# markweberdev/maskbit

Hardware: AMD Instinct MI355X
Metric: images/sec (256x256, 64-step MaskBit-12bit, CFG) (higher is better)
Workload: dtype f16

## Files before the change

### maskbit_amd/csrc/gemm_ht.hip

```cpp
#include <algorithm>

#include "mb_kernels.h"

namespace mb {

#define MB_SWZ(r) (((r) >> 1) & 7)

typedef int i32x4 __attribute__((ext_vector_type(4)));
typedef int i32x8 __attribute__((ext_vector_type(8)));
typedef h16 h16x16 __attribute__((ext_vector_type(16)));


template <int MT, int EPI, int XP = 0, bool SEQ = false, bool PAIR = false, int NS = 1>
__global__ __launch_bounds__(512, 2) void gemm_ht_kernel(GemmArgs a, int tiles_m, int tiles_n) {
  constexpr bool HN = NS > 1, QN = NS == 4;
  constexpr int NTW = 4 / NS;
  static_assert(NS == 1 || NS == 2 || NS == 4, "column split");
  static_assert(!HN || (SEQ && !PAIR && XP == 6 && EPI == EPI_RES_F32), "half-column tiles: plain sequence tiles with mini-tiles, residual epilogue");
  static_assert(!SEQ || MT == 8, "sequence-aligned tiles use the 256-row machinery");
  static_assert(XP == 0 || XP == 6, "fp16 K-tiles, optionally with mini-tiles");
  static_assert(!PAIR || SEQ, "pair tiles are sequence-aligned");
  constexpr bool MINI = XP == 6;
  static_assert(!MINI || SEQ, "mini-tile passes are written for sequence-aligned tiles");
  constexpr int MINI_A = 128 * 64, MINI_B = 256 * 64;
  constexpr bool PERSIST = true;
  constexpr int BM = 32 * MT, MH = MT / 2;
  constexpr int AH_ROWS = BM / 2;
  constexpr int AH_BYTES = AH_ROWS * 128, BH_BYTES = 128 * 128;
  constexpr int X_BYTES = SEQ ? 1024 : 0;
  constexpr int PAR_BYTES = 2 * AH_BYTES + 2 * BH_BYTES + X_BYTES;
  constexpr int MINI_OFF = 2 * PAR_BYTES;
  constexpr int A_INSTR = AH_ROWS / 8;
  extern __shared__ __attribute__((aligned(16))) char smem[];

  const int tid = threadIdx.x, lane = tid & 63;
  const int wave = __builtin_amdgcn_readfirstlane(tid >> 6);
  const int grp = wave >> 2;
  const int wm = wave >> 2, wn = wave & 3;
  const int l15 = lane & 15, g = lane >> 4;
  const int K = a.K, nk = K / 64;
  constexpr bool SPLIT = !PAIR;
  const int KA = SPLIT && a.kw ? a.kw : K, nka = KA / 64;
  const int KW = SPLIT && a.kw ? a.kw : K, nkw = KW / 64;
  const h16* const Alo = SPLIT && a.A2 ? a.A2 : a.A;
  const h16* const Wlo = a.W;
  const int SQ = a.seq_rows ? a.seq_rows : 257;
  const int tps_sh = 31 - __builtin_clz((unsigned)((SQ - 1) >> (PAIR ? 7 : 8)));
  const int TPS = 1 << tps_sh;
  const int ntiles = tiles_m * tiles_n;

  struct Plan {
    uint32_t offA[2][2], offB[2][2], offX;
    int m0, n0;
    int cls;
    int q;
    int seq;
    int hb;
  };
  int dstA[2], dstB[2];
#pragma unroll
  for (int j = 0; j < 2; ++j) { dstA[j] = min(wave + 8 * j, A_INSTR - 1) * 1024; dstB[j] = (QN ? (wave >> 1) * 4 + (wave & 1) : wave + 8 * j) * 1024; }
  auto make_plan = [&](int vb, Plan& p) {
    int lane_o = lane;
    asm volatile("" : "+v"(lane_o));
    const int L = xcd_remap(vb, ntiles);
    const int sr = L / (8 * tiles_n);
    const int rows_sr = min(8, tiles_m - sr * 8);
    const int rem = L - sr * 8 * tiles_n;
    const int tn = rem / rows_sr, tm = sr * 8 + (rem - tn * rows_sr);
    p.m0 = SEQ ? (tm >> tps_sh) * SQ + (tm & (TPS - 1)) * (PAIR ? 128 : 256) : tm * BM; p.n0 = (tn / NS) * 256;
    p.hb = tn % NS;
    p.cls = SEQ ? (tm >> tps_sh) * SQ + SQ - 1 : 0; p.q = SEQ ? tm & (TPS - 1) : 0;
    p.seq = SEQ ? tm >> tps_sh : tm;
#pragma unroll
    for (int j = 0; j < 2; ++j) {
      const int ja = min(wave + 8 * j, A_INSTR - 1);
      const int hra = ja * 8 + (lane_o >> 3);
      const int wms = hra / (8 * MT), r = hra - wms * (8 * MT);
      const int slot_a = (lane_o & 7) ^ MB_SWZ(hra);
      const int hrb = (QN ? (wave >> 1) * 4 + (wave & 1) : wave + 8 * j) * 8 + (lane_o >> 3);
      const int wns = hrb >> 5, c = hrb & 31;
      const int slot_b = (lane_o & 7) ^ MB_SWZ(hrb);
#pragma unroll
      for (int h = 0; h < 2; ++h) {
        const int gm = PAIR ? p.m0 + h * a.pair_rows + hra : min(p.m0 + wms * (16 * MT) + h * (8 * MT) + r, a.M - 1);
        p.offA[h][j] = (uint32_t)gm * (uint32_t)(2 * KA) + slot_a * 16;
        const int gn = min(p.n0 + wns * 64 + (HN ? p.hb * (64 / NS) : h * 32) + c, a.N - 1);
        p.offB[h][j] = (uint32_t)gn * (uint32_t)(2 * KW) + slot_b * 16;
      }
    }
    p.offX = (uint32_t)(PAIR ? p.cls + ((lane_o >> 3) == 1 ? a.pair_rows : 0) : min(p.cls, a.M - 1)) * (uint32_t)(2 * KA) + ((lane_o & 7) ^ MB_SWZ(lane_o >> 3)) * 16;
  };
  auto ktile_a = [&](int u) -> const char* { if constexpr (!SPLIT) return (const char*)a.A + u * 128; return (const char*)(u < nka ? a.A : Alo) + (u < nka ? u : u - nka) * 128; };
  auto ktile_w = [&](int u) -> const char* { if constexpr (!SPLIT) return (const char*)a.W + u * 128; return (const char*)(u < nkw ? a.W : Wlo) + (u < nkw ? u : u - nkw) * 128; };
  auto dma_x = [&](const Plan& p, const char* kp, int parb) {
    if (SEQ && wave == 7) MB_GLDS16_SB(kp, p.offX, smem + parb + 2 * AH_BYTES + 2 * BH_BYTES);
  };
  auto dma_a = [&](const Plan& p, const char* kp, int parb, int h) {
    char* buf = smem + parb + h * AH_BYTES;
#pragma unroll
    for (int j = 0; j < 2; ++j) {
      MB_GLDS16_SB2(kp, p.offA[h][j], buf, dstA[j]);
    }
  };
  auto dma_b = [&](const Plan& p, const char* kp, int parb, int h) {
    if (HN && h == 1) return;
    char* buf = smem + parb + 2 * AH_BYTES + h * BH_BYTES;
#pragma unroll
    for (int j = 0; j < (QN ? 1 : 2); ++j) {
      MB_GLDS16_SB2(kp, p.offB[h][j], buf, dstB[j]);
    }
  };
  const int KM = SPLIT && a.kw ? a.kw : K;
  const int nmk = KM / 128;
  const int nseq = PAIR ? a.pair_rows / SQ : a.M / SQ;
  const int grp_bytes = PAIR ? TPS * 128 : TPS * 256;
  const bool mini_every = MINI && (PAIR ? a.nlo == 2 : !a.kw);
  struct MiniPos { const uint8_t *a4, *w4, *xs, *ws; };
  const uint32_t ml_a = (uint32_t)((lane >> 2) * 2 * KM + (((lane & 3) ^ ((lane >> 3) & 3)) * 16));
  auto ml_w = [&]() -> uint32_t { int lo_ = lane; asm volatile("" : "+v"(lo_)); return (uint32_t)lo_ * 16; };
  const uint32_t ml_xs = (uint32_t)(lane >> 5) * (uint32_t)nseq * (uint32_t)grp_bytes + (lane & 15) * 4;
  auto ml_ws = [&]() -> uint32_t { int lo_ = lane; asm volatile("" : "+v"(lo_)); return (uint32_t)(lo_ & 15) * 4; };
  auto mini_pos = [&](const Plan& p) -> MiniPos {
    constexpr int si = 0, ps = 0;
    const int m0 = p.m0, n0 = p.n0, hb = p.hb, tq = p.q, sq = p.seq;
    const uint32_t row0 = PAIR ? m0 + wave * 16 : m0 + (wave >> 2) * 128 + ps * 64 + (wave & 3) * 16;
    const uint32_t wrow = QN ? wave * 4 + hb : HN ? (wave >> 1) * 4 + hb * 2 + (wave & 1) : wave;
    const uint32_t gq = PAIR ? tq * 2 + wm : tq * 4 + wm * 2 + ps;
    MiniPos m;
    m.a4 = a.lo[si].A4 + (size_t)row0 * 2 * KM;
    m.w4 = a.lo[si].W4 + (size_t)((n0 >> 4) + wrow) * nmk * 1024;
    m.xs = a.lo[si].a_scale + ((uint32_t)sq * (uint32_t)grp_bytes + gq * 64);
    m.ws = a.lo[si].w_scale + (uint32_t)(((n0 >> 6) + wn) * nmk) * 64;
    auto uni = [](const uint8_t* q) -> const uint8_t* {
      const uint64_t v = (uint64_t)q;
      return (const uint8_t*)(((uint64_t)(uint32_t)__builtin_amdgcn_readfirstlane((int)(v >> 32)) << 32) | (uint32_t)__builtin_amdgcn_readfirstlane((int)v));
    };
    m.a4 = uni(m.a4); m.w4 = uni(m.w4); m.xs = uni(m.xs); m.ws = uni(m.ws);
    return m;
  };
  const uint32_t xs_step = 2u * (uint32_t)nseq * (uint32_t)grp_bytes;
  auto mini_step = [&](MiniPos& m) { m.a4 += 64; m.w4 += 1024; m.xs += xs_step; m.ws += 64; };
  auto mini_switch = [&](MiniPos& m) {
    const size_t back = (size_t)nmk;
    if constexpr (PAIR) {
      auto ka = (const char __attribute__((address_space(4)))*)__builtin_amdgcn_kernarg_segment_ptr();
      asm volatile("" : "+s"(ka));
      auto l = (const GemmArgs::LoSet __attribute__((address_space(4)))*)(ka + offsetof(GemmArgs, lo));
      m.a4 += ((uintptr_t)l[1].A4 - (uintptr_t)l[0].A4) - back * 64;
      m.w4 += ((uintptr_t)l[1].W4 - (uintptr_t)l[0].W4) - back * 1024;
      m.xs += ((uintptr_t)l[1].a_scale - (uintptr_t)l[0].a_scale) - back * xs_step;
      m.ws += ((uintptr_t)l[1].w_scale - (uintptr_t)l[0].w_scale) - back * 64;
    } else {
      m.a4 += (size_t)64 * 2 * KM - back * 64;
      m.w4 -= back * 1024;
      m.xs += 64 - back * xs_step;
      m.ws -= back * 64;
    }
  };
  auto mini_dma_a = [&](const MiniPos& m) {
    MB_GLDS16_SB(m.a4, ml_a, smem + MINI_OFF + wave * 1024);
  };
  auto mini_dma_b = [&](const MiniPos& m) {
    if constexpr (QN) {
      if (wave < 4) MB_GLDS16_SB(m.w4, ml_w(), smem + MINI_OFF + MINI_A + wave * 1024);
      return;
    }
    if constexpr (HN) {
      MB_GLDS16_SB(m.w4, ml_w(), smem + MINI_OFF + MINI_A + wave * 1024);
      return;
    }
    const uint32_t mlw = ml_w();
#pragma unroll
    for (int jx = 0; jx < 2; ++jx)
      MB_GLDS16_SB(m.w4 + (size_t)(8 * jx) * nmk * 1024, mlw, smem + MINI_OFF + MINI_A + (wave + 8 * jx) * 1024);
  };
  int mws = 0, mxs = 0;
  auto mini_scale_issue = [&](const MiniPos& m) {
    asm volatile("global_load_dword %0, %1, %2" : "=v"(mxs) : "v"(ml_xs), "s"(m.xs) : "memory");
    asm volatile("global_load_dword %0, %1, %2" : "=v"(mws) : "v"(ml_ws()), "s"(m.ws) : "memory");
  };
  auto prologue_rest = [&](const Plan& p) {
    const char *a0 = ktile_a(0), *a1 = ktile_a(1), *w0 = ktile_w(0), *w1 = ktile_w(1);
    dma_a(p, a0, 0, 0); dma_b(p, w0, 0, 0); dma_b(p, w0, 0, 1); dma_a(p, a0, 0, 1);
    dma_a(p, a1, PAR_BYTES, 0); dma_b(p, w1, PAR_BYTES, 1); dma_a(p, a1, PAR_BYTES, 1); dma_b(p, w1, PAR_BYTES, 0);
  };
  auto prologue_x = [&](const Plan& p) { dma_x(p, ktile_a(0), 0); dma_x(p, ktile_a(1), PAR_BYTES); };
  auto prologue = [&](const Plan& p) { prologue_x(p); prologue_rest(p); if constexpr (MINI) { const MiniPos m0 = mini_pos(p); mini_dma_a(m0); mini_dma_b(m0); } };

  int foff[2], xoffe[2];
#pragma unroll
  for (int ks = 0; ks < 2; ++ks) {
    foff[ks] = l15 * 128 + (((ks * 4 + g) ^ MB_SWZ(l15)) * 16);
    xoffe[ks] = (l15 == 0 || (PAIR && l15 == 1)) ? 2 * AH_BYTES + 2 * BH_BYTES + foff[ks] : foff[ks];
  }
  const int mfo = (lane & 15) * 64 + (((lane >> 4) ^ ((lane >> 1) & 3)) * 16);
  const int xbase = wm * (8 * MT) * 128;
  const int wbase = 2 * AH_BYTES + wn * 32 * 128;

#define MB_LOAD_A(H)                                                                            \
  _Pragma("unroll") for (int i = 0; i < MH; ++i) _Pragma("unroll") for (int ks = 0; ks < 2; ++ks) \
      xa[i] = frag_set(xa[i], *(const h16x8*)(par + (H) * AH_BYTES + xbase + i * 16 * 128 + fo[ks]), ks);
#define MB_LOAD_B(H)                                                                            \
  _Pragma("unroll") for (int i = 0; i < (QN ? 1 : 2); ++i) _Pragma("unroll") for (int ks = 0; ks < 2; ++ks) \
      wb[H][i] = frag_set(wb[H][i], *(const h16x8*)(par + wbase + (H) * BH_BYTES + i * 16 * 128 + fo[ks]), ks);
#define MB_SYNC_L()                                     \
  __builtin_amdgcn_s_barrier();                         \
  __builtin_amdgcn_sched_barrier(0);                    \
  __builtin_amdgcn_s_setprio(1);
  auto frag_set = [](h16x16 f, h16x8 v, int ks) -> h16x16 {
    return ks == 0 ? __builtin_shufflevector(__builtin_shufflevector(v, v, 0, 1, 2, 3, 4, 5, 6, 7, 0, 1, 2, 3, 4, 5, 6, 7), f, 0, 1, 2, 3, 4, 5, 6, 7, 24, 25, 26, 27, 28, 29, 30, 31)
                   : __builtin_shufflevector(f, __builtin_shufflevector(v, v, 0, 1, 2, 3, 4, 5, 6, 7, 0, 1, 2, 3, 4, 5, 6, 7), 0, 1, 2, 3, 4, 5, 6, 7, 16, 17, 18, 19, 20, 21, 22, 23);
  };
  auto mma_tile = [&](f32x4 c, const h16x16& w, const h16x16& x) -> f32x4 {
    c = MB_MFMA_16x16x32(__builtin_shufflevector(w, w, 0, 1, 2, 3, 4, 5, 6, 7), __builtin_shufflevector(x, x, 0, 1, 2, 3, 4, 5, 6, 7), c);
    return MB_MFMA_16x16x32(__builtin_shufflevector(w, w, 8, 9, 10, 11, 12, 13, 14, 15), __builtin_shufflevector(x, x, 8, 9, 10, 11, 12, 13, 14, 15), c);
  };
#define MB_MMA_END                                                                                  \
  __builtin_amdgcn_s_setprio(0);                                                                    \
  __builtin_amdgcn_sched_barrier(0);                                                                \
  __builtin_amdgcn_s_barrier();
#define MB_MMA(AH, BH) MB_MMA_DO(AH, BH) MB_MMA_END
#define MB_MINI_ONE(AH, N, I)                                                                       \
  acc[N][(AH) * MH + (I)] = __builtin_amdgcn_mfma_scale_f32_16x16x128_f8f6f4(                        \
      __builtin_shufflevector(mwb[N], mwb[N], 0, 1, 2, 3, -1, -1, -1, -1), __builtin_shufflevector(mxa[I], mxa[I], 0, 1, 2, 3, -1, -1, -1, -1), \
      acc[N][(AH) * MH + (I)], 4, 4, N, mwsel, I, mxs);
#define MB_MINI_MMA_QN(AH)                                                                          \
  MB_MINI_ONE(AH, 0, 0) MB_MINI_ONE(AH, 0, 1) MB_MINI_ONE(AH, 0, 2) MB_MINI_ONE(AH, 0, 3)           \
  _Pragma("unroll") for (int i = 0; i < MH; ++i) asm volatile("" : "+v"(acc[0][(AH) * MH + i]));
#define MB_MINI_MMA_HN(AH)                                                                          \
  MB_MINI_ONE(AH, 0, 0) MB_MINI_ONE(AH, 1, 0) MB_MINI_ONE(AH, 0, 1) MB_MINI_ONE(AH, 1, 1)           \
  MB_MINI_ONE(AH, 0, 2) MB_MINI_ONE(AH, 1, 2) MB_MINI_ONE(AH, 0, 3) MB_MINI_ONE(AH, 1, 3)           \
  _Pragma("unroll") for (int i = 0; i < MH; ++i) _Pragma("unroll") for (int n = 0; n < 2; ++n)      \
    asm volatile("" : "+v"(acc[n][(AH) * MH + i]));
#define MB_MINI_MMA(AH)                                                                             \
  MB_MINI_ONE(AH, 0, 0) MB_MINI_ONE(AH, 1, 0) MB_MINI_ONE(AH, 2, 0) MB_MINI_ONE(AH, 3, 0)           \
  MB_MINI_ONE(AH, 0, 1) MB_MINI_ONE(AH, 1, 1) MB_MINI_ONE(AH, 2, 1) MB_MINI_ONE(AH, 3, 1)           \
  MB_MINI_ONE(AH, 0, 2) MB_MINI_ONE(AH, 1, 2) MB_MINI_ONE(AH, 2, 2) MB_MINI_ONE(AH, 3, 2)           \
  MB_MINI_ONE(AH, 0, 3) MB_MINI_ONE(AH, 1, 3) MB_MINI_ONE(AH, 2, 3) MB_MINI_ONE(AH, 3, 3)           \
  _Pragma("unroll") for (int i = 0; i < MH; ++i) _Pragma("unroll") for (int n = 0; n < 4; ++n)      \
    asm volatile("" : "+v"(acc[n][(AH) * MH + i]));
#define MB_MMA_DO(AH, BH)                                                                           \
  {                                                                                                 \
    _Pragma("unroll") for (int i = 0; i < MH; ++i) _Pragma("unroll") for (int n = 0; n < (QN ? 1 : 2); ++n)  \
      acc[(BH) * 2 + n][(AH) * MH + i] = mma_tile(acc[(BH) * 2 + n][(AH) * MH + i], wb[BH][n], xa[i]); \
  }

  Plan cur;
  int vb = blockIdx.x;
  make_plan(vb, cur);
  auto scales_load = [&](const Plan& p) {
    const MiniPos m0 = mini_pos(p);
    mws = *(const int*)(m0.ws + ml_ws());
    mxs = *(const int*)(m0.xs + ml_xs);
  };
  auto scales_pack = [&]() {
    if constexpr (MINI) { asm volatile("s_waitcnt vmcnt(0)" : "+v"(mws), "+v"(mxs) :: "memory"); return; }
  };
  if constexpr (MINI) scales_load(cur);
  prologue(cur);
  if constexpr (MINI) scales_pack();
  else asm volatile("s_waitcnt vmcnt(0)" ::: "memory");
  __builtin_amdgcn_s_barrier();

  while (true) {
    f32x4 acc[4][MT];
#pragma unroll
    for (int i = 0; i < 4; ++i)
#pragma unroll
      for (int j = 0; j < MT; ++j) acc[i][j] = f32x4{0.f, 0.f, 0.f, 0.f};
    f32x4 acce[2] = {f32x4{0.f, 0.f, 0.f, 0.f}, f32x4{0.f, 0.f, 0.f, 0.f}};
    const bool cls_on = __builtin_amdgcn_readfirstlane(cur.q) == TPS - 1;
    h16x16 xa[MH], wb[2][2];

    MiniPos mp = {};
    if constexpr (MINI) { mp = mini_pos(cur); mini_step(mp); }
    if (grp == 1) __builtin_amdgcn_s_barrier();
#define MB_KTILE MB_KTILE_(0)
#define MB_KTILE_(MAH)               \
    {                                                                                                    \
      const char* par = smem + parb; \
      int fo[2], xo[2]; \
      _Pragma("unroll") for (int ks = 0; ks < 2; ++ks) { fo[ks] = foff[ks]; xo[ks] = xoffe[ks]; } \
       \
       \
       \
      const bool n1 = t >= 1 && t + 1 < nk, n2 = t + 2 < nk; \
       \
      MB_LOAD_B(0) MB_LOAD_A(0)                           \
      h16x16 xe; \
      if (SEQ && wm == 0 && cls_on) { xe = frag_set(xe, *(const h16x8*)(par + xo[0]), 0); xe = frag_set(xe, *(const h16x8*)(par + xo[1]), 1); } \
      MB_SYNC_L() \
      if (SEQ && wm == 0 && cls_on) { _Pragma("unroll") for (int n = 0; n < (QN ? 1 : 2); ++n) acce[n] = mma_tile(acce[n], wb[0][n], xe); } \
      MB_MMA_DO(0, 0) MB_MMA_END \
       \
      if constexpr (!HN) { MB_LOAD_B(1) } \
      if (!HN && SEQ && wm == 1 && cls_on) { xe = frag_set(xe, *(const h16x8*)(par + xo[0]), 0); xe = frag_set(xe, *(const h16x8*)(par + xo[1]), 1); } \
       \
      const bool mini_issue = MINI && t >= 1 && mdue != 0; \
      if (MINI && mini_issue) { if (mj == nmk) mini_switch(mp); mini_scale_issue(mp); mini_dma_a(mp); } \
      if (n1) dma_a(cur, pa1, PAR_BYTES - parb, 1); \
      MB_SYNC_L() \
      if (!HN && SEQ && wm == 1 && cls_on) { _Pragma("unroll") for (int n = 0; n < 2; ++n) acce[n] = mma_tile(acce[n], wb[1][n], xe); } \
      if constexpr (!HN) { MB_MMA_DO(0, 1) } MB_MMA_END \
       \
      MB_LOAD_A(1) \
      if (MINI && mini_issue) { mini_dma_b(mp); mini_step(mp); ++mj; } \
      if (n2) dma_a(cur, pa2, parb, 0); \
      MB_SYNC_L() if (!HN) { MB_MMA_DO(1, 1) } MB_MMA_END \
       \
       \
       \
      if (n2) { dma_b(cur, pw2, parb, 1); dma_x(cur, pa2, parb); dma_b(cur, pw2, parb, 0); } \
      if (t >= 1) { \
        if (MINI) {                                \
           \
           \
          const int wsel = __builtin_amdgcn_readfirstlane(n2 ? (wave == 7 ? 2 : 1) : 0); \
          if constexpr (QN)                               \
            asm volatile("s_cmp_eq_u32 %[w], 0\n\ts_cbranch_scc1 1f\n\ts_cmp_eq_u32 %[w], 1\n\ts_cbranch_scc1 2f\n\ts_waitcnt vmcnt(4)\n\ts_branch 3f\n" \
                         "1:\n\ts_waitcnt vmcnt(0)\n\ts_branch 3f\n2:\n\ts_waitcnt vmcnt(3)\n3:" \
                         : "+v"(mxs), "+v"(mws) : [w] "s"(wsel) : "memory", "scc"); \
          else if constexpr (HN)                          \
            asm volatile("s_cmp_eq_u32 %[w], 0\n\ts_cbranch_scc1 1f\n\ts_cmp_eq_u32 %[w], 1\n\ts_cbranch_scc1 2f\n\ts_waitcnt vmcnt(5)\n\ts_branch 3f\n" \
                         "1:\n\ts_waitcnt vmcnt(0)\n\ts_branch 3f\n2:\n\ts_waitcnt vmcnt(4)\n3:" \
                         : "+v"(mxs), "+v"(mws) : [w] "s"(wsel) : "memory", "scc"); \
          else \
          asm volatile("s_cmp_eq_u32 %[w], 0\n\ts_cbranch_scc1 1f\n\ts_cmp_eq_u32 %[w], 1\n\ts_cbranch_scc1 2f\n\ts_waitcnt vmcnt(7)\n\ts_branch 3f\n" \
                       "1:\n\ts_waitcnt vmcnt(0)\n\ts_branch 3f\n2:\n\ts_waitcnt vmcnt(6)\n3:" \
                       : "+v"(mxs), "+v"(mws) : [w] "s"(wsel) : "memory", "scc"); \
        } else if (n2) {                                  \
          if (SEQ && wave == 7) asm volatile("s_waitcnt vmcnt(7)" ::: "memory"); \
          else asm volatile("s_waitcnt vmcnt(6)" ::: "memory"); \
        } else asm volatile("s_waitcnt vmcnt(0)" ::: "memory"); \
      } \
      MB_SYNC_L() MB_MMA_DO(1, 0) MB_MMA_END \
       \
      if constexpr (MINI) { \
        if (mrun != 0) { \
          int mfo_ = mfo; \
          asm volatile("" : "+v"(mfo_)); \
          const char* mbuf = smem + MINI_OFF + mfo_; \
          i32x4 mxa[4], mwb[4]; \
          _Pragma("unroll") for (int n = 0; n < NTW; ++n) mwb[n] = *(const i32x4*)(mbuf + MINI_A + (wn * (64 / NS) + n * 16) * 64); \
          _Pragma("unroll") for (int i = 0; i < 4; ++i) mxa[i] = *(const i32x4*)(mbuf + (wm * 64 + i * 16) * 64); \
          const int mwsel = HN ? (int)((uint32_t)mws >> ((32 / NS) * cur.hb)) : mws;    \
          MB_SYNC_L() \
          if constexpr (QN) { MB_MINI_MMA_QN(MAH) } else if constexpr (HN) { MB_MINI_MMA_HN(MAH) } else { MB_MINI_MMA(MAH) } \
           \
          asm volatile("s_nop 15\n\ts_nop 15" ::: "memory"); \
          MB_MMA_END \
        } \
      } \
       \
      pa1 = pa2; \
      pa2 = SPLIT && t + 3 == nka ? (const char*)Alo : pa2 + 128; \
      pw2 = SPLIT && t + 3 == nkw ? (const char*)Wlo : pw2 + 128; \
      parb = PAR_BYTES - parb; \
      mdue ^= mflip; mrun ^= mflip; \
    }
    {
      int t = 0;
      int parb = 0;
      const char *pa1 = ktile_a(1), *pa2 = ktile_a(2), *pw2 = ktile_w(2);
      const int mflip = mini_every ? 0 : 1;
      int mdue = 1, mrun = mini_every ? 1 : 0, mj = 1;
      (void)mj;
      if constexpr (MINI && !PAIR) {
        for (; t < nk / 2; ++t) MB_KTILE_(0)
        for (; t < nk; ++t) MB_KTILE_(1)
      } else {
        for (; t < nk; ++t) MB_KTILE
      }
    }
#undef MB_KTILE
#undef MB_KTILE_
    if (grp == 0) __builtin_amdgcn_s_barrier();

    const float* __restrict__ resp = a.residual;
    float* __restrict__ out32 = a.out_f32;
    h16* __restrict__ out16 = a.out_h16;
    const int m0 = cur.m0, n0 = cur.n0, clsrow = cur.cls, tq = cur.q;
    constexpr int NROWS = SEQ ? MT + 1 : MT;
    int l15e = l15, ge = g;
    asm volatile("" : "+v"(l15e), "+v"(ge));
    auto row_of = [&](int r) {
      if (PAIR) return r < MT ? m0 + (r / MH) * a.pair_rows + wm * 64 + (r % MH) * 16 + l15e : clsrow + (l15e == 1 ? a.pair_rows : 0);
      return r < MT ? m0 + wm * (16 * MT) + (r / MH) * (8 * MT) + (r % MH) * 16 + l15e : clsrow;
    };
    auto col_of = [&](int r, int nt) {
      if (HN) return n0 + wn * 64 + cur.hb * (64 / NS) + (nt & (NTW - 1)) * 16 + ge * 4;
      return r < MT ? n0 + wn * 64 + (nt >> 1) * 32 + (nt & 1) * 16 + ge * 4 : n0 + wn * 64 + wm * 32 + nt * 16 + ge * 4;
    };
    auto row_ok = [&](int r) {
      if (PAIR) return r < MT ? true : (l15e < 2 && tq == TPS - 1);
      return r < MT ? row_of(r) < (SEQ ? m0 + 256 : a.M) : (l15e == 0 && (!HN || wm == 0) && tq == TPS - 1);
    };
    const int nvb = vb + gridDim.x;
    const bool has_next = PERSIST && nvb < ntiles;
    Plan nxt;
    if (has_next) { make_plan(nvb, nxt); prologue_x(nxt); }
    f32x4 bias4[4], bcls[2];
    if constexpr (MINI) {
#pragma unroll
      for (int nt = 0; nt < 4; ++nt) bias4[nt] = *(const f32x4*)(a.bias + col_of(0, nt));
      if (SEQ) { bcls[0] = *(const f32x4*)(a.bias + col_of(MT, 0)); bcls[1] = *(const f32x4*)(a.bias + col_of(MT, 1)); }
      else { bcls[0] = bias4[0]; bcls[1] = bias4[1]; }
      if (has_next) scales_load(nxt);
      asm volatile("s_waitcnt vmcnt(0)" : "+v"(bias4[0]), "+v"(bias4[1]), "+v"(bias4[2]), "+v"(bias4[3]), "+v"(bcls[0]), "+v"(bcls[1]) :: "memory");
      if (has_next) scales_pack();
      if (has_next) { prologue_rest(nxt); const MiniPos m0 = mini_pos(nxt); mini_dma_a(m0); mini_dma_b(m0); }
    } else {
#define MB_LDG16(dst, ptr) asm volatile("global_load_dwordx4 %0, %1, off" : "=v"(dst) : "v"(ptr) : "memory")
#pragma unroll
    for (int nt = 0; nt < 4; ++nt) MB_LDG16(bias4[nt], a.bias + col_of(0, nt));
    if (SEQ) { MB_LDG16(bcls[0], a.bias + col_of(MT, 0)); MB_LDG16(bcls[1], a.bias + col_of(MT, 1)); }
    else { bcls[0] = bias4[0]; bcls[1] = bias4[1]; }
#undef MB_LDG16
    if (has_next) prologue_rest(nxt);
    {
      const int hn = __builtin_amdgcn_readfirstlane(has_next ? 1 : 0);
      asm volatile("s_cmp_lg_u32 %[hn], 0\n\ts_cbranch_scc1 1f\n\ts_waitcnt vmcnt(0)\n1:\n\ts_waitcnt vmcnt(16)"
                   : "+v"(bias4[0]), "+v"(bias4[1]), "+v"(bias4[2]), "+v"(bias4[3]), "+v"(bcls[0]), "+v"(bcls[1])
                   : [hn] "s"(hn) : "memory", "scc");
    }
    }

    if constexpr (PAIR) {
      const float osc = a.scale ? *a.scale : 1.0f;
      auto pair2 = [&](f32x4& c, f32x4& dl, const f32x4& b) {
        f32x4 vc = __builtin_elementwise_fma(c, (f32x4)(osc), b);
        f32x4 vu = __builtin_elementwise_fma(dl, (f32x4)(osc), vc);
        if (EPI == EPI_GELU_H16 || EPI == EPI_GELU_F32) {
          const f32x2 c0 = gelu_erf2((f32x2){vc[0], vc[1]}), c1 = gelu_erf2((f32x2){vc[2], vc[3]});
          const f32x2 u0 = gelu_erf2((f32x2){vu[0], vu[1]}), u1 = gelu_erf2((f32x2){vu[2], vu[3]});
          vc = f32x4{c0.x, c0.y, c1.x, c1.y};
          vu = f32x4{u0.x - c0.x, u0.y - c0.y, u1.x - c1.x, u1.y - c1.y};
        }
        c = vc; dl = vu;
        asm volatile("" : "+v"(c), "+v"(dl));
      };
#pragma unroll
      for (int i = 0; i < MH; ++i)
#pragma unroll
        for (int nt = 0; nt < 4; ++nt) pair2(acc[nt][i], acc[nt][i + MH], bias4[nt]);
#pragma unroll
      for (int n = 0; n < 2; ++n) {
        f32x4 cup;
#pragma unroll
        for (int e = 0; e < 4; ++e) cup[e] = __shfl_up(acce[n][e], 1);
        f32x4 c = l15e == 1 ? cup : acce[n], dl = l15e == 1 ? acce[n] : f32x4{0.f, 0.f, 0.f, 0.f};
        pair2(c, dl, bcls[n]);
        acce[n] = l15e == 1 ? dl : c;
      }
    } else {
      const float osc = a.scale ? *a.scale : 1.0f;
#pragma unroll
      for (int r = 0; r < NROWS; ++r) {
        const int nn = r < MT ? NTW : (QN ? 1 : 2);
#pragma unroll
        for (int nt = 0; nt < nn; ++nt) {
          f32x4& c = r < MT ? acc[nt][r < MT ? r : 0] : acce[nt & 1];
          c = __builtin_elementwise_fma(c, (f32x4)(osc), r < MT ? bias4[nt] : bcls[nt & 1]);
          if (EPI == EPI_GELU_H16 || EPI == EPI_GELU_F32) {
            const f32x2 lo = gelu_erf2((f32x2){c[0], c[1]}), hi = gelu_erf2((f32x2){c[2], c[3]});
            c[0] = lo.x; c[1] = lo.y; c[2] = hi.x; c[3] = hi.y;
          }
          asm volatile("" : "+v"(c));
        }
      }
    }
    if (has_next) asm volatile("s_waitcnt vmcnt(0)" ::: "memory");
    if constexpr (SEQ && EPI == EPI_GELU_H16) {
      if (a.out4) {
        const uint32_t blk = (uint32_t)(n0 >> 6) + wn;
        const uint32_t nsq = (uint32_t)(PAIR ? a.pair_rows : a.M) / (uint32_t)SQ;
        const uint32_t ngrp = (uint32_t)TPS * (PAIR ? 2 : 4);
        auto emit4 = [&](uint32_t p0, uint32_t p1, uint32_t p2, uint32_t p3, uint8_t* dst, uint32_t row) {
          const auto sw = __builtin_amdgcn_permlane16_swap((p0 & 0xffffu) | (p2 << 16), (p1 & 0xffffu) | (p3 << 16), false, false);
          const uint32_t q0 = __builtin_amdgcn_perm(sw[1], sw[0], 0x05040100u);
          const uint32_t q1 = __builtin_amdgcn_perm(sw[1], sw[0], 0x07060302u);
          const auto sx = __builtin_amdgcn_permlane32_swap(q0, q1, false, false);
          *(uint2*)(dst + (size_t)row * 2 * a.N + ((n0 + wn * 64) >> 1) + (ge >> 1) * 16 + (ge & 1) * 8) = make_uint2(sx[0], sx[1]);
        };
#pragma unroll
        for (int hh = 0; hh < (PAIR ? 1 : 2); ++hh) {
          uint32_t sc4 = 0, sl4 = 0;
#pragma unroll
          for (int ii = 0; ii < MH; ++ii) {
            const int i = hh * MH + ii;
            float am = 0.f;
#pragma unroll
            for (int nt = 0; nt < 4; ++nt)
#pragma unroll
              for (int e = 0; e < 4; ++e) am = fmaxf(am, fabsf(acc[nt][i][e]));
            am = rows_max(am);
            const float mul = fp4_scale_mul_nosat(am);
            const uint32_t row = (uint32_t)row_of(i);
            sc4 |= fp4_scale_byte_nosat(am) << (8 * ii);
            emit4(fp4_pack4(acc[0][i][0], acc[0][i][1], acc[0][i][2], acc[0][i][3], mul), fp4_pack4(acc[1][i][0], acc[1][i][1], acc[1][i][2], acc[1][i][3], mul),
                  fp4_pack4(acc[2][i][0], acc[2][i][1], acc[2][i][2], acc[2][i][3], mul), fp4_pack4(acc[3][i][0], acc[3][i][1], acc[3][i][2], acc[3][i][3], mul),
                  a.out4, row);
            if (a.out4l) {
              f32x4 l[4];
              float aml = 0.f;
#pragma unroll
              for (int nt = 0; nt < 4; ++nt)
#pragma unroll
                for (int e = 0; e < 4; ++e) { l[nt][e] = acc[nt][i][e] - (float)to_h(acc[nt][i][e]); aml = fmaxf(aml, fabsf(l[nt][e])); }
              aml = rows_max(aml);
              const float mull = fp4_scale_mul_nosat(aml);
              sl4 |= fp4_scale_byte_nosat(aml) << (8 * ii);
              emit4(fp4_pack4(l[0][0], l[0][1], l[0][2], l[0][3], mull), fp4_pack4(l[1][0], l[1][1], l[1][2], l[1][3], mull),
                    fp4_pack4(l[2][0], l[2][1], l[2][2], l[2][3], mull), fp4_pack4(l[3][0], l[3][1], l[3][2], l[3][3], mull), a.out4l, row);
            }
          }
          const uint32_t gq = PAIR ? (uint32_t)tq * 2 + wm : (uint32_t)tq * 4 + wm * 2 + hh;
          if (ge == 0) ((uint32_t*)a.out4_scale)[((blk * nsq + (uint32_t)cur.seq) * ngrp + gq) * 16 + l15e] = sc4;
          if (ge == 0 && a.out4l) ((uint32_t*)a.out4l_scale)[((blk * nsq + (uint32_t)cur.seq) * ngrp + gq) * 16 + l15e] = sl4;
        }
      }
    }
    if (EPI == EPI_RES_F32) {
      const bool lnres = a.ln_stats != nullptr;
      constexpr int RB = (PAIR && MINI) ? 1 : 2;
      constexpr int NB = MT / RB;
      static_assert(MT % RB == 0, "whole batches");
      constexpr int NQ = QN ? 1 : 2;
      float4 rv[RB][2];
      float2 sv[RB] = {};
      auto fetch = [&](int k) {
        const int p = k / NB, r0 = (k % NB) * RB;
#pragma unroll
        for (int j = 0; j < RB; ++j) {
          const uint32_t rowc = (uint32_t)min(row_of(r0 + j), a.M - 1);
#pragma unroll
          for (int q = 0; q < NQ; ++q) rv[j][q] = *(const float4*)((const char*)resp + (size_t)((rowc * (uint32_t)a.N + (uint32_t)col_of(r0 + j, 2 * p + q)) * 4u));
          if (lnres) sv[j] = *(const float2*)(a.ln_stats + 2 * (size_t)rowc);
        }
      };
      auto add_one = [&](f32x4& c, const float4& rr, const float2& st, const f32x4& gm, const f32x4& bt) {
        if (lnres) {
          c[0] += ln_affine(rr.x, st.x, st.y, gm[0], bt[0]); c[1] += ln_affine(rr.y, st.x, st.y, gm[1], bt[1]);
          c[2] += ln_affine(rr.z, st.x, st.y, gm[2], bt[2]); c[3] += ln_affine(rr.w, st.x, st.y, gm[3], bt[3]);
        } else { c[0] += rr.x; c[1] += rr.y; c[2] += rr.z; c[3] += rr.w; }
      };
      f32x4 gm[2] = {}, bt[2] = {};
      auto affine = [&](int p) {
        if (lnres) {
#pragma unroll
          for (int q = 0; q < NQ; ++q) { gm[q] = *(const f32x4*)(a.ln_g + col_of(0, 2 * p + q)); bt[q] = *(const f32x4*)(a.ln_b + col_of(0, 2 * p + q)); }
        }
      };
      auto add = [&](int k) {
        const int p = k / NB, r0 = (k % NB) * RB;
#pragma unroll
        for (int j = 0; j < RB; ++j)
#pragma unroll
          for (int q = 0; q < NQ; ++q) add_one(acc[2 * p + q][r0 + j], rv[j][q], sv[j], gm[q], bt[q]);
      };
      auto store_one = [&](const f32x4& c, int r, int nt) {
        *(float4*)((char*)out32 + (size_t)(((uint32_t)row_of(r) * (uint32_t)a.N + (uint32_t)col_of(r, nt)) * 4u)) = make_float4(c[0], c[1], c[2], c[3]);
      };
      auto store = [&](int k) {
        const int p = k / NB, r0 = (k % NB) * RB;
#pragma unroll
        for (int j = 0; j < RB; ++j)
          if (row_ok(r0 + j)) {
#pragma unroll
            for (int q = 0; q < NQ; ++q) store_one(acc[2 * p + q][r0 + j], r0 + j, 2 * p + q);
          }
      };
      affine(0);
      fetch(0);
      constexpr int NSWEEP = HN ? 1 : 2;
#pragma unroll
      for (int k = 0; k < NSWEEP * NB; ++k) {
        asm volatile("" ::: "memory");
        add(k);
        if (k + 1 < NSWEEP * NB) { if ((k + 1) % NB == 0) affine((k + 1) / NB); fetch(k + 1); }
        asm volatile("" ::: "memory");
        store(k);
      }
      if (SEQ) {
        float4 rr[2]; float2 st = {};
        const uint32_t rowc = (uint32_t)min(row_of(MT), a.M - 1);
#pragma unroll
        for (int q = 0; q < NQ; ++q) {
          rr[q] = *(const float4*)((const char*)resp + (size_t)((rowc * (uint32_t)a.N + (uint32_t)col_of(MT, q)) * 4u));
          if (lnres) { gm[q] = *(const f32x4*)(a.ln_g + col_of(MT, q)); bt[q] = *(const f32x4*)(a.ln_b + col_of(MT, q)); }
        }
        if (lnres) st = *(const float2*)(a.ln_stats + 2 * (size_t)rowc);
#pragma unroll
        for (int q = 0; q < NQ; ++q) add_one(acce[q], rr[q], st, gm[q], bt[q]);
        if (row_ok(MT)) {
#pragma unroll
          for (int q = 0; q < NQ; ++q) store_one(acce[q], MT, q);
        }
      }
    } else {
      float satm = 0.f;
      bool satnan = false;
#pragma unroll
      for (int r = 0; r < NROWS; ++r) {
        const bool ok = row_ok(r);
        const int nn = r < MT ? 4 : 2;
        if (EPI == EPI_H16 || EPI == EPI_GELU_H16) {
#pragma unroll
          for (int pr = 0; pr < nn / 2; ++pr) {
            const f32x4 ca = r < MT ? acc[2 * pr][r < MT ? r : 0] : acce[0];
            const f32x4 cb = r < MT ? acc[2 * pr + 1][r < MT ? r : 0] : acce[1];
            if (a.sat && ok) {
              satm = fmaxf(fmaxf(satm, fmaxf(fmaxf(fabsf(ca[0]), fabsf(ca[1])), fmaxf(fabsf(ca[2]), fabsf(ca[3])))),
                           fmaxf(fmaxf(fabsf(cb[0]), fabsf(cb[1])), fmaxf(fabsf(cb[2]), fabsf(cb[3]))));
              const float sm = (ca[0] + ca[1]) + (ca[2] + ca[3]) + (cb[0] + cb[1]) + (cb[2] + cb[3]);
              satnan |= sm != sm;
            }
            const h16x2 ta0 = {to_h(ca[0]), to_h(ca[1])}, ta1 = {to_h(ca[2]), to_h(ca[3])};
            const h16x2 tb0 = {to_h(cb[0]), to_h(cb[1])}, tb1 = {to_h(cb[2]), to_h(cb[3])};
            const auto s0 = __builtin_amdgcn_permlane16_swap(__builtin_bit_cast(uint32_t, ta0), __builtin_bit_cast(uint32_t, tb0), false, false);
            const auto s1 = __builtin_amdgcn_permlane16_swap(__builtin_bit_cast(uint32_t, ta1), __builtin_bit_cast(uint32_t, tb1), false, false);
            const int n = col_of(r, 2 * pr + (ge & 1)) - (ge & 1) * 4;
            const size_t ob = (size_t)(((uint32_t)row_of(r) * (uint32_t)a.N + (uint32_t)n) * 2u);
            if (ok) *(uint4*)((char*)out16 + ob) = make_uint4(s0[0], s1[0], s0[1], s1[1]);
          }
        } else if (ok) {
#pragma unroll
          for (int nt = 0; nt < 4; ++nt)
            if (nt < nn) {
              const f32x4 c = r < MT ? acc[nt][r < MT ? r : 0] : acce[nt & 1];
              *(float4*)((char*)out32 + (size_t)(((uint32_t)row_of(r) * (uint32_t)a.N + (uint32_t)col_of(r, nt)) * 4u)) = make_float4(c[0], c[1], c[2], c[3]);
            }
        }
      }
      if ((EPI == EPI_H16 || EPI == EPI_GELU_H16) && a.sat && (satnan || !(satm <= MB_H16_MAX))) atomicAdd(a.sat, 1u);
    }
    if (has_next) __builtin_amdgcn_s_barrier();
    if (!has_next) break;
    cur = nxt;
    vb = nvb;
  }
#undef MB_LOAD_A
#undef MB_LOAD_B
#undef MB_SYNC_L
#undef MB_MMA
#undef MB_MMA_DO
#undef MB_MMA_END
#undef MB_MINI_ONE
#undef MB_MINI_MMA
#undef MB_MINI_MMA_HN
#undef MB_MINI_MMA_QN
}

static int g_cu_override = 0;
void set_cu_count(int n) { g_cu_override = n > 0 ? n : 0; }
static int num_cu_cached() {
  static int num_cu = 0;
  if (g_cu_override) return g_cu_override;
  if (!num_cu) {
    int dev = 0;
    (void)hipGetDevice(&dev);
    (void)hipDeviceGetAttribute(&num_cu, hipDeviceAttributeMultiprocessorCount, dev);
    if (num_cu <= 0) num_cu = 256;
  }
  return num_cu;
}

template <int MT, int EPI, int XP = 0, bool SEQ = false, bool PAIR = false, int NS = 1>
static void launch_ht(hipStream_t s, const GemmArgs& a, bool persistent = true) {
  constexpr int BM = 32 * MT;
  constexpr int LDS = 2 * (BM * 128 + 2 * 128 * 128 + (SEQ ? 1024 : 0)) + (XP == 6 ? 128 * 64 + 256 * 64 : 0);
  static bool configured = false;
  if (!configured) {
    (void)hipFuncSetAttribute((const void*)gemm_ht_kernel<MT, EPI, XP, SEQ, PAIR, NS>, hipFuncAttributeMaxDynamicSharedMemorySize, LDS);
    configured = true;
  }
  const int sq_rows = a.seq_rows ? a.seq_rows : 257;
  const int tiles_m = PAIR ? (a.pair_rows / sq_rows) * ((sq_rows - 1) / 128) : (SEQ ? (a.M / sq_rows) * ((sq_rows - 1) / 256) : (a.M + BM - 1) / BM), tiles_n = (a.N / 256) * NS;
  const int grid = persistent ? std::min(tiles_m * tiles_n, num_cu_cached()) : tiles_m * tiles_n;
  hipLaunchKernelGGL((gemm_ht_kernel<MT, EPI, XP, SEQ, PAIR, NS>), dim3(grid), dim3(512), LDS, s, a, tiles_m, tiles_n);
}

bool gemm_ht_supported(GemmEpi epi, const GemmArgs& a) {
  const int sqr = a.seq_rows ? a.seq_rows : 257;
  const int tok = a.pair_rows ? 128 : 256;
  if (a.seq_rows && ((sqr - 1) % tok || ((sqr - 1) / tok & ((sqr - 1) / tok - 1)) || (!a.pair_rows && a.M % sqr))) return false;
  if (a.pair_rows && (a.pair_rows % sqr || a.M != 2 * a.pair_rows || a.A2 || a.kw || epi == EPI_GELU_F32)) return false;
  if (a.nlo && (a.nlo > 2 || (a.pair_rows ? a.pair_rows % sqr : a.M % sqr) || (a.kw ? a.kw : a.K) % 128 || (!a.pair_rows && a.nlo != 1) ||
                ((a.A2 || a.kw) && (a.pair_rows || !a.A2 || a.K != 2 * a.kw)) ||
                !a.lo[0].A4 || !a.lo[0].W4 || !a.lo[0].a_scale || !a.lo[0].w_scale ||
                (a.nlo == 2 && (!a.lo[1].A4 || !a.lo[1].W4 || !a.lo[1].a_scale || !a.lo[1].w_scale)) || (uint64_t)a.M * a.K * 2 >= (1ull << 32) ||
                epi == EPI_GELU_F32)) return false;
  return epi != EPI_LOGITS_F32 && a.N % 256 == 0 && a.K % 64 == 0 && a.K >= 128 && (a.M >= 512 || a.nlo) &&
         (uint64_t)a.M * a.K * 2 < (1ull << 32) && (uint64_t)a.N * a.K * 2 < (1ull << 32) &&
         (uint64_t)a.M * a.N * 4 < (1ull << 32);
}

void gemm_ht(hipStream_t s, GemmEpi epi, const GemmArgs& a, int mt) {
  bool persistent = true;
  const int sqr = a.seq_rows ? a.seq_rows : 257;
  const long seq_tiles = (long)(a.M / sqr) * ((sqr - 1) / 256);
  if (mt >= 1000) { persistent = false; mt -= 1000; }
  if (mt != 6 && mt != 8 && mt != 257) {
    const int num_cu = num_cu_cached();
    auto cost = [&](int m) {
      const long tiles = (long)((a.M + 32 * m - 1) / (32 * m)) * (a.N / 256);
      return (double)((tiles + num_cu - 1) / num_cu) * 32 * m * (m == 8 ? 1.0 : 1.04);
    };
    mt = cost(8) <= cost(6) ? 8 : 6;
    if (a.M % sqr == 0) {
      const long tiles = (long)(a.M / sqr) * ((sqr - 1) / 256) * (a.N / 256);
      if ((double)((tiles + num_cu - 1) / num_cu) * 272 < cost(mt)) mt = 257;
    }
  }
  if (a.nlo) {
    switch (epi) {
      case EPI_H16: if (a.pair_rows) launch_ht<8, EPI_H16, 6, true, true>(s, a, persistent); else launch_ht<8, EPI_H16, 6, true>(s, a, persistent); break;
      case EPI_GELU_H16: if (a.pair_rows) launch_ht<8, EPI_GELU_H16, 6, true, true>(s, a, persistent); else launch_ht<8, EPI_GELU_H16, 6, true>(s, a, persistent); break;
      case EPI_RES_F32:
        if (a.pair_rows) launch_ht<8, EPI_RES_F32, 6, true, true>(s, a, persistent);
        else if (seq_tiles * (a.N / 256) * 4 <= num_cu_cached()) launch_ht<8, EPI_RES_F32, 6, true, false, 4>(s, a, persistent);
        else if (seq_tiles * (a.N / 256) * 2 <= num_cu_cached()) launch_ht<8, EPI_RES_F32, 6, true, false, 2>(s, a, persistent);
        else launch_ht<8, EPI_RES_F32, 6, true>(s, a, persistent);
        break;
      default: break;
    }
    return;
  }
  if (a.pair_rows) {
    switch (epi) {
      case EPI_H16: launch_ht<8, EPI_H16, 0, true, true>(s, a, persistent); break;
      case EPI_GELU_H16: launch_ht<8, EPI_GELU_H16, 0, true, true>(s, a, persistent); break;
      case EPI_RES_F32: launch_ht<8, EPI_RES_F32, 0, true, true>(s, a, persistent); break;
      default: break;
    }
    return;
  }
#define MB_HT_CASE(E)                                                      \
  case E:                                                                  \
    if (mt == 257) launch_ht<8, E, 0, true>(s, a, persistent);             \
    else if (mt == 8) launch_ht<8, E>(s, a, persistent);                   \
    else launch_ht<6, E>(s, a, persistent);                                \
    break;
  switch (epi) {
    MB_HT_CASE(EPI_H16) MB_HT_CASE(EPI_GELU_H16) MB_HT_CASE(EPI_RES_F32) MB_HT_CASE(EPI_GELU_F32)
    default: break;
  }
#undef MB_HT_CASE
}

}
```

Before: 34.70.

## Pipeline fp16 epilogue row by row with direct stores and relaxed waits

For sequence-aligned fp16 and GELU-fp16 epilogues, bias, GELU, optional fp4 packing and the fp16 stores now run row by row. Stores go out through inline global_store with scalar base pointers and permlane16 swaps that build 16-byte writes. The full vmcnt(0) wait before the epilogue becomes a computed partial wait, so next-tile prefetch loads keep flowing while stores drain. This cuts epilogue latency and register pressure, but relies on exact hand-counted vmcnt values, and the CLS bias now comes from bias4 instead of separate loads.

```diff
diff --git a/maskbit_amd/csrc/gemm_ht.hip b/maskbit_amd/csrc/gemm_ht.hip
--- a/maskbit_amd/csrc/gemm_ht.hip
+++ b/maskbit_amd/csrc/gemm_ht.hip
@@ -6,6 +6,7 @@
 
 #define MB_SWZ(r) (((r) >> 1) & 7)
 
+typedef int i32x2 __attribute__((ext_vector_type(2)));
 typedef int i32x4 __attribute__((ext_vector_type(4)));
 typedef int i32x8 __attribute__((ext_vector_type(8)));
 typedef h16 h16x16 __attribute__((ext_vector_type(16)));
@@ -21,6 +22,7 @@
   static_assert(XP == 0 || XP == 6, "fp16 K-tiles, optionally with mini-tiles");
   static_assert(!PAIR || SEQ, "pair tiles are sequence-aligned");
   constexpr bool MINI = XP == 6;
+  constexpr bool ROWPIPE = SEQ && (EPI == EPI_H16 || EPI == EPI_GELU_H16);
   static_assert(!MINI || SEQ, "mini-tile passes are written for sequence-aligned tiles");
   constexpr int MINI_A = 128 * 64, MINI_B = 256 * 64;
   constexpr bool PERSIST = true;
@@ -72,6 +74,10 @@
     p.hb = tn % NS;
     p.cls = SEQ ? (tm >> tps_sh) * SQ + SQ - 1 : 0; p.q = SEQ ? tm & (TPS - 1) : 0;
     p.seq = SEQ ? tm >> tps_sh : tm;
+    if constexpr (ROWPIPE) {
+      p.m0 = __builtin_amdgcn_readfirstlane(p.m0); p.n0 = __builtin_amdgcn_readfirstlane(p.n0); p.cls = __builtin_amdgcn_readfirstlane(p.cls);
+      p.q = __builtin_amdgcn_readfirstlane(p.q); p.seq = __builtin_amdgcn_readfirstlane(p.seq);
+    }
 #pragma unroll
     for (int j = 0; j < 2; ++j) {
       const int ja = min(wave + 8 * j, A_INSTR - 1);
@@ -404,7 +410,7 @@
     if constexpr (MINI) {
 #pragma unroll
       for (int nt = 0; nt < 4; ++nt) bias4[nt] = *(const f32x4*)(a.bias + col_of(0, nt));
-      if (SEQ) { bcls[0] = *(const f32x4*)(a.bias + col_of(MT, 0)); bcls[1] = *(const f32x4*)(a.bias + col_of(MT, 1)); }
+      if (SEQ && !ROWPIPE) { bcls[0] = *(const f32x4*)(a.bias + col_of(MT, 0)); bcls[1] = *(const f32x4*)(a.bias + col_of(MT, 1)); }
       else { bcls[0] = bias4[0]; bcls[1] = bias4[1]; }
       if (has_next) scales_load(nxt);
       asm volatile("s_waitcnt vmcnt(0)" : "+v"(bias4[0]), "+v"(bias4[1]), "+v"(bias4[2]), "+v"(bias4[3]), "+v"(bcls[0]), "+v"(bcls[1]) :: "memory");
@@ -414,7 +420,7 @@
 #define MB_LDG16(dst, ptr) asm volatile("global_load_dwordx4 %0, %1, off" : "=v"(dst) : "v"(ptr) : "memory")
 #pragma unroll
     for (int nt = 0; nt < 4; ++nt) MB_LDG16(bias4[nt], a.bias + col_of(0, nt));
-    if (SEQ) { MB_LDG16(bcls[0], a.bias + col_of(MT, 0)); MB_LDG16(bcls[1], a.bias + col_of(MT, 1)); }
+    if (SEQ && !ROWPIPE) { MB_LDG16(bcls[0], a.bias + col_of(MT, 0)); MB_LDG16(bcls[1], a.bias + col_of(MT, 1)); }
     else { bcls[0] = bias4[0]; bcls[1] = bias4[1]; }
 #undef MB_LDG16
     if (has_next) prologue_rest(nxt);
@@ -426,24 +432,28 @@
     }
     }
 
-    if constexpr (PAIR) {
-      const float osc = a.scale ? *a.scale : 1.0f;
-      auto pair2 = [&](f32x4& c, f32x4& dl, const f32x4& b) {
-        f32x4 vc = __builtin_elementwise_fma(c, (f32x4)(osc), b);
-        f32x4 vu = __builtin_elementwise_fma(dl, (f32x4)(osc), vc);
-        if (EPI == EPI_GELU_H16 || EPI == EPI_GELU_F32) {
-          const f32x2 c0 = gelu_erf2((f32x2){vc[0], vc[1]}), c1 = gelu_erf2((f32x2){vc[2], vc[3]});
-          const f32x2 u0 = gelu_erf2((f32x2){vu[0], vu[1]}), u1 = gelu_erf2((f32x2){vu[2], vu[3]});
-          vc = f32x4{c0.x, c0.y, c1.x, c1.y};
-          vu = f32x4{u0.x - c0.x, u0.y - c0.y, u1.x - c1.x, u1.y - c1.y};
-        }
-        c = vc; dl = vu;
-        asm volatile("" : "+v"(c), "+v"(dl));
-      };
-#pragma unroll
-      for (int i = 0; i < MH; ++i)
-#pragma unroll
-        for (int nt = 0; nt < 4; ++nt) pair2(acc[nt][i], acc[nt][i + MH], bias4[nt]);
+    const float osc = a.scale ? *a.scale : 1.0f;
+    auto pair2 = [&](f32x4& c, f32x4& dl, const f32x4& b) {
+      f32x4 vc = __builtin_elementwise_fma(c, (f32x4)(osc), b);
+      f32x4 vu = __builtin_elementwise_fma(dl, (f32x4)(osc), vc);
+      if (EPI == EPI_GELU_H16 || EPI == EPI_GELU_F32) {
+        const f32x2 c0 = gelu_erf2((f32x2){vc[0], vc[1]}), c1 = gelu_erf2((f32x2){vc[2], vc[3]});
+        const f32x2 u0 = gelu_erf2((f32x2){vu[0], vu[1]}), u1 = gelu_erf2((f32x2){vu[2], vu[3]});
+        vc = f32x4{c0.x, c0.y, c1.x, c1.y};
+        vu = f32x4{u0.x - c0.x, u0.y - c0.y, u1.x - c1.x, u1.y - c1.y};
+      }
+      c = vc; dl = vu;
+      asm volatile("" : "+v"(c), "+v"(dl));
+    };
+    auto plain1 = [&](f32x4& c, const f32x4& b) {
+      c = __builtin_elementwise_fma(c, (f32x4)(osc), b);
+      if (EPI == EPI_GELU_H16 || EPI == EPI_GELU_F32) {
+        const f32x2 lo = gelu_erf2((f32x2){c[0], c[1]}), hi = gelu_erf2((f32x2){c[2], c[3]});
+        c[0] = lo.x; c[1] = lo.y; c[2] = hi.x; c[3] = hi.y;
+      }
+      asm volatile("" : "+v"(c));
+    };
+    auto pair_cls = [&]() {
 #pragma unroll
       for (int n = 0; n < 2; ++n) {
         f32x4 cup;
@@ -453,75 +463,131 @@
         pair2(c, dl, bcls[n]);
         acce[n] = l15e == 1 ? dl : c;
       }
+    };
+    (void)pair2; (void)plain1; (void)pair_cls;
+    if constexpr (ROWPIPE) {
+      constexpr int NE4 = PAIR ? MH + 1 : MT + 2;
+      const bool o4 = EPI == EPI_GELU_H16 && a.out4 != nullptr, o4l = o4 && a.out4l != nullptr;
+      float satm = 0.f;
+      bool satnan = false;
+      auto store16 = [&](int r, int pr, const f32x4& ca, const f32x4& cb, bool lane_ok) {
+        if (a.sat && lane_ok) {
+          satm = fmaxf(fmaxf(satm, fmaxf(fmaxf(fabsf(ca[0]), fabsf(ca[1])), fmaxf(fabsf(ca[2]), fabsf(ca[3])))),
+                       fmaxf(fmaxf(fabsf(cb[0]), fabsf(cb[1])), fmaxf(fabsf(cb[2]), fabsf(cb[3]))));
+          const float sm = (ca[0] + ca[1]) + (ca[2] + ca[3]) + (cb[0] + cb[1]) + (cb[2] + cb[3]);
+          satnan |= sm != sm;
+        }
+        const h16x2 ta0 = {to_h(ca[0]), to_h(ca[1])}, ta1 = {to_h(ca[2]), to_h(ca[3])};
+        const h16x2 tb0 = {to_h(cb[0]), to_h(cb[1])}, tb1 = {to_h(cb[2]), to_h(cb[3])};
+        const auto s0 = __builtin_amdgcn_permlane16_swap(__builtin_bit_cast(uint32_t, ta0), __builtin_bit_cast(uint32_t, tb0), false, false);
+        const auto s1 = __builtin_amdgcn_permlane16_swap(__builtin_bit_cast(uint32_t, ta1), __builtin_bit_cast(uint32_t, tb1), false, false);
+        const int n = col_of(r, 2 * pr + (ge & 1)) - (ge & 1) * 4;
+        const uint32_t ob = ((uint32_t)row_of(r) * (uint32_t)a.N + (uint32_t)n) * 2u;
+        const i32x4 v = {(int)s0[0], (int)s1[0], (int)s0[1], (int)s1[1]};
+        if (lane_ok) asm volatile("s_nop 4\n\tglobal_store_dwordx4 %0, %1, %2\n\ts_nop 1" :: "v"(ob), "v"(v), "s"(out16) : "memory");
+      };
+      const uint32_t blk = (uint32_t)(n0 >> 6) + wn;
+      const uint32_t nsq = (uint32_t)(PAIR ? a.pair_rows : a.M) / (uint32_t)SQ;
+      const uint32_t ngrp = (uint32_t)TPS * (PAIR ? 2 : 4);
+      auto emit4 = [&](uint32_t p0, uint32_t p1, uint32_t p2, uint32_t p3, uint8_t* dst, uint32_t row) {
+        const auto sw = __builtin_amdgcn_permlane16_swap((p0 & 0xffffu) | (p2 << 16), (p1 & 0xffffu) | (p3 << 16), false, false);
+        const uint32_t q0 = __builtin_amdgcn_perm(sw[1], sw[0], 0x05040100u);
+        const uint32_t q1 = __builtin_amdgcn_perm(sw[1], sw[0], 0x07060302u);
+        const auto sx = __builtin_amdgcn_permlane32_swap(q0, q1, false, false);
+        const uint32_t ob = row * 2u * (uint32_t)a.N + (uint32_t)(((n0 + wn * 64) >> 1) + (ge >> 1) * 16 + (ge & 1) * 8);
+        const i32x2 v = {(int)sx[0], (int)sx[1]};
+        asm volatile("s_nop 4\n\tglobal_store_dwordx2 %0, %1, %2" :: "v"(ob), "v"(v), "s"(dst) : "memory");
+      };
+      uint32_t sc4 = 0, sl4 = 0;
+      auto e2m1_row = [&](int i) {
+        const int ii = i % MH;
+        float am = 0.f;
+#pragma unroll
+        for (int nt = 0; nt < 4; ++nt)
+#pragma unroll
+          for (int e = 0; e < 4; ++e) am = fmaxf(am, fabsf(acc[nt][i][e]));
+        am = rows_max(am);
+        const float mul = fp4_scale_mul_nosat(am);
+        const uint32_t row = (uint32_t)row_of(i);
+        sc4 |= fp4_scale_byte_nosat(am) << (8 * ii);
+        emit4(fp4_pack4(acc[0][i][0], acc[0][i][1], acc[0][i][2], acc[0][i][3], mul), fp4_pack4(acc[1][i][0], acc[1][i][1], acc[1][i][2], acc[1][i][3], mul),
+              fp4_pack4(acc[2][i][0], acc[2][i][1], acc[2][i][2], acc[2][i][3], mul), fp4_pack4(acc[3][i][0], acc[3][i][1], acc[3][i][2], acc[3][i][3], mul),
+              a.out4, row);
+        if (o4l) {
+          f32x4 l[4];
+          float aml = 0.f;
+#pragma unroll
+          for (int nt = 0; nt < 4; ++nt)
+#pragma unroll
+            for (int e = 0; e < 4; ++e) { l[nt][e] = acc[nt][i][e] - (float)to_h(acc[nt][i][e]); aml = fmaxf(aml, fabsf(l[nt][e])); }
+          aml = rows_max(aml);
+          const float mull = fp4_scale_mul_nosat(aml);
+          sl4 |= fp4_scale_byte_nosat(aml) << (8 * ii);
+          emit4(fp4_pack4(l[0][0], l[0][1], l[0][2], l[0][3], mull), fp4_pack4(l[1][0], l[1][1], l[1][2], l[1][3], mull),
+                fp4_pack4(l[2][0], l[2][1], l[2][2], l[2][3], mull), fp4_pack4(l[3][0], l[3][1], l[3][2], l[3][3], mull), a.out4l, row);
+        }
+        if (ii == MH - 1) {
+          const int hh = i / MH;
+          const uint32_t gq = PAIR ? (uint32_t)tq * 2 + wm : (uint32_t)tq * 4 + wm * 2 + hh;
+          const uint32_t sb = (((blk * nsq + (uint32_t)cur.seq) * ngrp + gq) * 16 + l15e) * 4u;
+          if (ge == 0) asm volatile("s_nop 4\n\tglobal_store_dword %0, %1, %2" :: "v"(sb), "v"(sc4), "s"(a.out4_scale) : "memory");
+          if (o4l) { if (ge == 0) asm volatile("s_nop 4\n\tglobal_store_dword %0, %1, %2" :: "v"(sb), "v"(sl4), "s"(a.out4l_scale) : "memory"); }
+          sc4 = 0; sl4 = 0;
+        }
+      };
+#pragma unroll
+      for (int i = 0; i < (PAIR ? MH : MT); ++i) {
+#pragma unroll
+        for (int nt = 0; nt < 4; ++nt) {
+          if constexpr (PAIR) pair2(acc[nt][i], acc[nt][i + MH], bias4[nt]);
+          else plain1(acc[nt][i], bias4[nt]);
+        }
+        if (o4) e2m1_row(i);
+#pragma unroll
+        for (int pr = 0; pr < 2; ++pr) store16(i, pr, acc[2 * pr][i], acc[2 * pr + 1][i], true);
+        if constexpr (PAIR) {
+#pragma unroll
+          for (int pr = 0; pr < 2; ++pr) store16(i + MH, pr, acc[2 * pr][i + MH], acc[2 * pr + 1][i + MH], true);
+        }
+      }
+      if (cls_on) {
+        bcls[0] = wm ? bias4[2] : bias4[0]; bcls[1] = wm ? bias4[3] : bias4[1];
+        if constexpr (PAIR) pair_cls();
+        else { plain1(acce[0], bcls[0]); plain1(acce[1], bcls[1]); }
+        store16(MT, 0, acce[0], acce[1], PAIR ? l15e < 2 : l15e == 0);
+      }
+      if (has_next) {
+        const int wsel = __builtin_amdgcn_readfirstlane((cls_on ? 1 : 0) + (o4 ? (o4l ? 4 : 2) : 0));
+        asm volatile("s_cmp_eq_u32 %[w], 0\n\ts_cbranch_scc1 10f\n\ts_cmp_eq_u32 %[w], 1\n\ts_cbranch_scc1 11f\n\t"
+                     "s_cmp_eq_u32 %[w], 2\n\ts_cbranch_scc1 12f\n\ts_cmp_eq_u32 %[w], 3\n\ts_cbranch_scc1 13f\n\t"
+                     "s_cmp_eq_u32 %[w], 4\n\ts_cbranch_scc1 14f\n\t"
+                     "s_waitcnt vmcnt(%[c5])\n\ts_branch 19f\n"
+                     "10:\n\ts_waitcnt vmcnt(%[c0])\n\ts_branch 19f\n11:\n\ts_waitcnt vmcnt(%[c1])\n\ts_branch 19f\n"
+                     "12:\n\ts_waitcnt vmcnt(%[c2])\n\ts_branch 19f\n13:\n\ts_waitcnt vmcnt(%[c3])\n\ts_branch 19f\n"
+                     "14:\n\ts_waitcnt vmcnt(%[c4])\n19:"
+                     :: [w] "s"(wsel), [c0] "n"(16), [c1] "n"(17), [c2] "n"(16 + NE4), [c3] "n"(17 + NE4), [c4] "n"(16 + 2 * NE4), [c5] "n"(17 + 2 * NE4)
+                     : "memory", "scc");
+      }
+      if (a.sat && (satnan || !(satm <= MB_H16_MAX))) atomicAdd(a.sat, 1u);
     } else {
-      const float osc = a.scale ? *a.scale : 1.0f;
-#pragma unroll
-      for (int r = 0; r < NROWS; ++r) {
-        const int nn = r < MT ? NTW : (QN ? 1 : 2);
-#pragma unroll
-        for (int nt = 0; nt < nn; ++nt) {
-          f32x4& c = r < MT ? acc[nt][r < MT ? r : 0] : acce[nt & 1];
-          c = __builtin_elementwise_fma(c, (f32x4)(osc), r < MT ? bias4[nt] : bcls[nt & 1]);
-          if (EPI == EPI_GELU_H16 || EPI == EPI_GELU_F32) {
-            const f32x2 lo = gelu_erf2((f32x2){c[0], c[1]}), hi = gelu_erf2((f32x2){c[2], c[3]});
-            c[0] = lo.x; c[1] = lo.y; c[2] = hi.x; c[3] = hi.y;
-          }
-          asm volatile("" : "+v"(c));
-        }
-      }
-    }
-    if (has_next) asm volatile("s_waitcnt vmcnt(0)" ::: "memory");
-    if constexpr (SEQ && EPI == EPI_GELU_H16) {
-      if (a.out4) {
-        const uint32_t blk = (uint32_t)(n0 >> 6) + wn;
-        const uint32_t nsq = (uint32_t)(PAIR ? a.pair_rows : a.M) / (uint32_t)SQ;
-        const uint32_t ngrp = (uint32_t)TPS * (PAIR ? 2 : 4);
-        auto emit4 = [&](uint32_t p0, uint32_t p1, uint32_t p2, uint32_t p3, uint8_t* dst, uint32_t row) {
-          const auto sw = __builtin_amdgcn_permlane16_swap((p0 & 0xffffu) | (p2 << 16), (p1 & 0xffffu) | (p3 << 16), false, false);
-          const uint32_t q0 = __builtin_amdgcn_perm(sw[1], sw[0], 0x05040100u);
-          const uint32_t q1 = __builtin_amdgcn_perm(sw[1], sw[0], 0x07060302u);
-          const auto sx = __builtin_amdgcn_permlane32_swap(q0, q1, false, false);
-          *(uint2*)(dst + (size_t)row * 2 * a.N + ((n0 + wn * 64) >> 1) + (ge >> 1) * 16 + (ge & 1) * 8) = make_uint2(sx[0], sx[1]);
-        };
-#pragma unroll
-        for (int hh = 0; hh < (PAIR ? 1 : 2); ++hh) {
-          uint32_t sc4 = 0, sl4 = 0;
-#pragma unroll
-          for (int ii = 0; ii < MH; ++ii) {
-            const int i = hh * MH + ii;
-            float am = 0.f;
-#pragma unroll
-            for (int nt = 0; nt < 4; ++nt)
-#pragma unroll
-              for (int e = 0; e < 4; ++e) am = fmaxf(am, fabsf(acc[nt][i][e]));
-            am = rows_max(am);
-            const float mul = fp4_scale_mul_nosat(am);
-            const uint32_t row = (uint32_t)row_of(i);
-            sc4 |= fp4_scale_byte_nosat(am) << (8 * ii);
-            emit4(fp4_pack4(acc[0][i][0], acc[0][i][1], acc[0][i][2], acc[0][i][3], mul), fp4_pack4(acc[1][i][0], acc[1][i][1], acc[1][i][2], acc[1][i][3], mul),
-                  fp4_pack4(acc[2][i][0], acc[2][i][1], acc[2][i][2], acc[2][i][3], mul), fp4_pack4(acc[3][i][0], acc[3][i][1], acc[3][i][2], acc[3][i][3], mul),
-                  a.out4, row);
-            if (a.out4l) {
-              f32x4 l[4];
-              float aml = 0.f;
-#pragma unroll
-              for (int nt = 0; nt < 4; ++nt)
-#pragma unroll
-                for (int e = 0; e < 4; ++e) { l[nt][e] = acc[nt][i][e] - (float)to_h(acc[nt][i][e]); aml = fmaxf(aml, fabsf(l[nt][e])); }
-              aml = rows_max(aml);
-              const float mull = fp4_scale_mul_nosat(aml);
-              sl4 |= fp4_scale_byte_nosat(aml) << (8 * ii);
-              emit4(fp4_pack4(l[0][0], l[0][1], l[0][2], l[0][3], mull), fp4_pack4(l[1][0], l[1][1], l[1][2], l[1][3], mull),
-                    fp4_pack4(l[2][0], l[2][1], l[2][2], l[2][3], mull), fp4_pack4(l[3][0], l[3][1], l[3][2], l[3][3], mull), a.out4l, row);
-            }
-          }
-          const uint32_t gq = PAIR ? (uint32_t)tq * 2 + wm : (uint32_t)tq * 4 + wm * 2 + hh;
-          if (ge == 0) ((uint32_t*)a.out4_scale)[((blk * nsq + (uint32_t)cur.seq) * ngrp + gq) * 16 + l15e] = sc4;
-          if (ge == 0 && a.out4l) ((uint32_t*)a.out4l_scale)[((blk * nsq + (uint32_t)cur.seq) * ngrp + gq) * 16 + l15e] = sl4;
-        }
-      }
-    }
-    if (EPI == EPI_RES_F32) {
+      if constexpr (PAIR) {
+#pragma unroll
+        for (int i = 0; i < MH; ++i)
+#pragma unroll
+          for (int nt = 0; nt < 4; ++nt) pair2(acc[nt][i], acc[nt][i + MH], bias4[nt]);
+        pair_cls();
+      } else {
+#pragma unroll
+        for (int r = 0; r < NROWS; ++r) {
+          const int nn = r < MT ? NTW : (QN ? 1 : 2);
+#pragma unroll
+          for (int nt = 0; nt < nn; ++nt) plain1(r < MT ? acc[nt][r < MT ? r : 0] : acce[nt & 1], r < MT ? bias4[nt] : bcls[nt & 1]);
+        }
+      }
+      if (has_next) asm volatile("s_waitcnt vmcnt(0)" ::: "memory");
+    }
+    if constexpr (ROWPIPE) {
+    } else if (EPI == EPI_RES_F32) {
       const bool lnres = a.ln_stats != nullptr;
       constexpr int RB = (PAIR && MINI) ? 1 : 2;
       constexpr int NB = MT / RB;
```

After: 34.92 (median of 6 runs). No clear change (+0.6%).
